# erhant/halo2-vectordb

Hardware: AMD Instinct MI355X
Metric: constraints/sec, proving hot path (witness+layout+commit MSM+NTT), kmeans k=16 circuit (higher is better)
Workload: dtype u32x8 (BN254 Fr/Fq, 254-bit Montgomery)

## Files before the change

halo2_vectordb_amd/csrc/field.hpp:

```cpp
#pragma once
#include <hip/hip_runtime.h>
#include <stdint.h>

#define HD __host__ __device__ __forceinline__

namespace vdb {

struct alignas(16) u256 {
  uint32_t w[8];
};

struct FrParams {
  static constexpr uint32_t P[8] = {0xf0000001u, 0x43e1f593u, 0x79b97091u, 0x2833e848u, 0x8181585du, 0xb85045b6u, 0xe131a029u, 0x30644e72u};
  static constexpr uint32_t R1[8] = {0x4ffffffbu, 0xac96341cu, 0x9f60cd29u, 0x36fc7695u, 0x7879462eu, 0x666ea36fu, 0x9a07df2fu, 0x0e0a77c1u};
  static constexpr uint32_t R2[8] = {0xae216da7u, 0x1bb8e645u, 0xe35c59e3u, 0x53fe3ab1u, 0x53bb8085u, 0x8c49833du, 0x7f4e44a5u, 0x0216d0b1u};
  static constexpr uint32_t INV = 0xefffffffu;
  static constexpr uint32_t P29[9] = {0x10000001u, 0x1f0fac9fu, 0x0e5c2450u, 0x07d090f3u, 0x1585d283u, 0x02db40c0u, 0x00a6e141u, 0x0e5c2634u, 0x0030644eu};
  static constexpr uint32_t INV29 = 0x0fffffffu;
};
struct FqParams {
  static constexpr uint32_t P[8] = {0xd87cfd47u, 0x3c208c16u, 0x6871ca8du, 0x97816a91u, 0x8181585du, 0xb85045b6u, 0xe131a029u, 0x30644e72u};
  static constexpr uint32_t R1[8] = {0xc58f0d9du, 0xd35d438du, 0xf5c70b3du, 0x0a78eb28u, 0x7879462cu, 0x666ea36fu, 0x9a07df2fu, 0x0e0a77c1u};
  static constexpr uint32_t R2[8] = {0x538afa89u, 0xf32cfc5bu, 0xd44501fbu, 0xb5e71911u, 0x0a417ff6u, 0x47ab1effu, 0xcab8351fu, 0x06d89f71u};
  static constexpr uint32_t INV = 0xe4866389u;
// ... 274 lines not shown
  uint64_t acc = 0;
#pragma unroll
  for (int k = 7; k < 18; k++) {
#pragma unroll
    for (int i = (k > 8 ? k - 8 : 0); i <= (k < 8 ? k : 8); i++) mad64(acc, WQ[i], V[k - i]);
    if (k >= 9) q[k - 9] = k < 17 ? ((uint32_t)acc & MASK) : (uint32_t)acc;
    acc >>= 29;
  }
  acc = 0;
#pragma unroll
  for (int k = 0; k < 9; k++) {
#pragma unroll
    for (int i = 0; i <= k; i++) {
      mad64(acc, W[i], V[k - i]);
      mad64(acc, q[i], NP[k - i]);
    }
    out[k] = (uint32_t)acc & MASK;
    acc >>= 29;
  }
#endif
}

template <class M>
HD void mont_sqr_core29(uint32_t out[9], const uint32_t A[9]) {
#if defined(__HIP_DEVICE_COMPILE__)
  uint32_t D[9];
#pragma unroll
  for (int j = 0; j < 9; j++) D[j] = A[j] << 1;
  asm(
#include "core29_sqr.inc"
// ... 216 lines not shown
```

halo2_vectordb_amd/csrc/gen_core29.py:

```python
#!/usr/bin/env python3
ACC = 30


def emit(name, pairs_of, n_arrays):
    O = lambda i: f"%{i}"
    base_p = 9 + 9 * n_arrays
    P = lambda j: f"%{base_p + j}"
    INV = f"%{base_p + 9}"
    acc, lo = f"v[{ACC}:{ACC + 1}]", f"v{ACC}"
    L, first = [], True
    for k in range(18):
        terms = list(pairs_of(k))
        js = range(1, k + 1) if k < 9 else range(k - 8, 9)
        terms += [(O(k - j), P(j)) for j in js]
        for x, y in terms:
            L.append(f"v_mad_u64_u32 {acc}, vcc, {x}, {y}, {0 if first else acc}")
            first = False
        if k < 9:
            L += [f"v_mul_lo_u32 {O(k)}, {lo}, {INV}", f"v_and_b32 {O(k)}, 0x1fffffff, {O(k)}", f"v_mad_u64_u32 {acc}, vcc, {O(k)}, {P(0)}, {acc}"]
        else:
            L.append(f"v_and_b32 {O(k - 9)}, 0x1fffffff, {lo}" if k < 17 else f"v_mov_b32 {O(k - 9)}, {lo}")
        if k < 17:
            L.append(f"v_lshrrev_b64 {acc}, 29, {acc}")
    with open(name, "w") as f:
# ... 32 lines not shown
            L.append(f"v_mad_u64_u32 {acc}, vcc, {W(i)}, {V(k - i)}, {0 if first else acc}")
            first = False
            L.append(f"v_mad_u64_u32 {acc}, vcc, {Q(i)}, {NP(k - i)}, {acc}")
        L.append(f"v_and_b32 {T(k)}, 0x1fffffff, {lo}")
        if k < 8:
            L.append(f"v_lshrrev_b64 {acc}, 29, {acc}")
    with open(name, "w") as f:
        f.write(f"// generated by gen_core29.py — {len(L)} instructions\n")
        f.write("\n".join('"%s\\n\\t"' % x for x in L) + "\n")
    return len(L)


print(emit_shoup("core29_shoup.inc"))


def emit_redc(name):
    O = lambda i: f"%{i}"
    T = lambda i: f"%{9 + i}"
    P = lambda j: f"%{18 + j}"
    INV = "%27"
    acc, lo = f"v[{ACC}:{ACC + 1}]", f"v{ACC}"
    L = []
    for k in range(18):
        if k < 9:
            L.append(f"v_mad_u64_u32 {acc}, vcc, {T(k)}, 1, {0 if k == 0 else acc}")
        js = range(1, k + 1) if k < 9 else range(k - 8, 9)
        for j in js:
            L.append(f"v_mad_u64_u32 {acc}, vcc, {O(k - j)}, {P(j)}, {acc}")
        if k < 9:
            L += [f"v_mul_lo_u32 {O(k)}, {lo}, {INV}", f"v_and_b32 {O(k)}, 0x1fffffff, {O(k)}", f"v_mad_u64_u32 {acc}, vcc, {O(k)}, {P(0)}, {acc}"]
# ... 12 lines not shown
```

halo2_vectordb_amd/csrc/limb9.hpp:

```cpp
#pragma once
#include <math.h>

#include "field.hpp"

namespace vdb {

struct L9 {
  uint32_t l[9];
};
HD L9 l9_split(const u256& a) {
  L9 r;
#pragma unroll
  for (int k = 0; k < 9; k++) {
    int pb = 29 * k, wb = pb >> 5, ob = pb & 31;
    uint32_t lo = a.w[wb];
    uint32_t hi = wb + 1 < 8 ? a.w[wb + 1 < 8 ? wb + 1 : 0] : 0u;
    r.l[k] = ob ? ((lo >> ob) | (hi << (32 - ob))) : lo;
    if (k < 8) r.l[k] &= 0x1fffffffu;
  }
  return r;
}
HD L9 l9_split32(const u256& a) {
  L9 r;
  r.l[0] = (a.w[0] << 5) & 0x1fffffffu;
// ... 79 lines not shown
  const u256 p = mod_p<Fr>();
  u256 r = w;
#pragma unroll
  for (int k = 8; k >= 0; k--) {
    uint32_t d = 0;
    for (int j = 28; j >= 0; j--) {
      u256 s, t;
      u256_add(s, r, r);
      const uint32_t borrow = u256_sub(t, s, p);
      r = borrow ? s : t;
      d |= (borrow ^ 1u) << j;
    }
    out[9 + k] = d;
  }
}
template <class M>
HD L9 l9_mul2(const L9& a1, const L9& b1, const L9& a2, const L9& b2) {
  L9 r;
  mont_core29_2<M>(r.l, a1.l, b1.l, a2.l, b2.l);
  return r;
}
template <class M>
HD L9 l9_sqr(const L9& a) {
  L9 r;
  mont_sqr_core29<M>(r.l, a.l);
  return r;
}
template <class M>
HD u256 l9_canon(const L9& t) {
  return lazy_canon<M>(l9_pack(t));
// ... 32 lines not shown
#pragma unroll
  for (int k = 0; k < 9; k++) {
    const uint32_t nk = (k == 0 ? 0x20000000u : 0x1fffffffu) - FrParams::P29[k];
    acc += (uint64_t)x.l[k] + (uint64_t)q * nk;
    x.l[k] = (uint32_t)acc & 0x1fffffffu;
    acc >>= 29;
  }
  u256 v = l9_pack(x), t, p2, pp = mod_p<Fr>();
  u256_add(p2, pp, pp);
  uint32_t keep = u256_sub(t, v, p2);
#pragma unroll
  for (int i = 0; i < 8; i++) v.w[i] = keep ? v.w[i] : t.w[i];
  return lazy_canon<Fr>(v);
}

}
```

halo2_vectordb_amd/csrc/ntt.hip:

```cpp
#include <type_traits>
#include <vector>

#include "common.hpp"
#include "limb9.hpp"
#include "shoup_tables.hpp"

namespace vdb {

#define NTT_THREADS 256
#define NTT_TILE 1024
#define NTT_MAX_PASSES 4
#define NTT_DEFAULT_COLGROUP 0x7fffffffu

struct NttPass {
  uint32_t log_n, S, log_inner, logG;
  uint32_t nprev;
  uint32_t prevS[NTT_MAX_PASSES];
  uint32_t first;
  uint32_t coset;
  uint32_t vslots;
  const u256* in_tab[4];
  uint32_t coset_out;
  uint32_t scale;
  uint32_t s0;
// ... 65 lines not shown
template <uint32_t CS, uint32_t s, uint32_t step, class F>
__device__ __forceinline__ void ntt_static_steps(F&& f) {
  if constexpr (s < CS) {
    f(std::integral_constant<uint32_t, s>{}, std::integral_constant<uint32_t, step>{});
    ntt_static_steps<CS, (s + 1 < CS ? s + 2 : s + 1), step + 1>(f);
  }
}
constexpr uint32_t ntt_spec_sh_res_log(uint32_t cs, bool sa) { return cs == 8 ? 0u : (sa ? 1u : 2u); }
template <bool LAST, bool VS = false, uint32_t CS = 0, uint32_t CS0 = 0, uint32_t CREN = 0, bool SA = false>
__global__ __launch_bounds__(NTT_THREADS) void k_ntt_pass(const u256* __restrict__ in, u256* __restrict__ out,
                                                         const u256* __restrict__ tw, const u256* __restrict__ tw_inter, NttPass p,
                                                         uint32_t tiles_per_col) {
  extern __shared__ uint4 smem[];
  constexpr bool SPEC = CS > 0;
  static_assert(!SA || ((CS == 8 || CS == 9) && !VS), "SA: the 256- and 512-point instantiations, not the virtual-column one");
  const uint32_t S = SPEC ? CS : p.S, P_logG = SPEC ? 10u - CS : p.logG, P_s0 = SPEC ? CS0 : p.s0, P_ren_mask = SPEC ? CREN : p.ren_mask;
  const uint32_t P_sh_res_log = SPEC ? ntt_spec_sh_res_log(CS, SA) : p.sh_res_log, P_sh_ns = SPEC ? ((1u << (CS ? CS - 1 : 0)) >> ntt_spec_sh_res_log(CS, SA)) : p.sh_ns;
  const int32_t P_sh_max_s = SPEC ? (int32_t)CS - 2 - (int32_t)ntt_spec_sh_res_log(CS, SA) : p.sh_max_s;
  const bool P_shoup = SPEC ? true : p.sh_tab != nullptr, P_blk0 = SPEC ? true : p.blk0 != 0;
  const uint32_t m = 1u << S, G = 1u << P_logG, T = m * G;
  const uint32_t row = m + 1, NE = G * row, NW = SA ? 0u : (m / 2 ? m / 2 : 1);
  L9Planes D, W;
  D.a = smem;
  D.b = D.a + NE;
  W.a = D.b + NE;
  W.b = W.a + NW;
  const uint32_t NS = P_shoup ? P_sh_ns : 0;
  L9Planes WS, WQ;
  WS.a = W.b + NW;
  WS.b = WS.a + NS;
  WQ.a = WS.b + NS;
// ... 75 lines not shown
    if (!LAST) {
      g = e & (G - 1);
      j = e >> P_logG;
    } else {
      j = e & (mload - 1);
      g = e / mload;
    }
    uint64_t idx = base + j * jstride + g * gstride;
    L9 v;
    if (!p.first || idx < p.in_len) {
      v = l9_split(from_src ? colsrc_fetch(csrc, idx, 1ull << p.log_n, p.n_blind) : ld256(cin + idx));
      if constexpr (VS) {
        v = l9_mul(v, l9_split(ld256(ctab + idx)));
      } else if (SA && p.coset) {
        const uint32_t r3 = (uint32_t)(idx % 3);
        if (r3 == 1) v = l9_mul_shoup<Fr>(v, kconst(p.zsh[1]), kconst(p.zsh[1] + 9));
        else if (r3 == 2) v = l9_mul_shoup<Fr>(v, kconst(p.zsh[2]), kconst(p.zsh[2] + 9));
        else if (p.coset == 2) v = l9_mul_shoup<Fr>(v, kconst(p.zsh[0]), kconst(p.zsh[0] + 9));
      } else if (p.coset) {
        uint32_t r3 = (uint32_t)(idx % 3);
        if (r3 == 1) v = l9_mul(v, Z1);
        else if (r3 == 2) v = l9_mul(v, Z2);
        else if (p.coset == 2) v = l9_mul(v, Z0);
      }
    } else {
#pragma unroll
      for (int k = 0; k < 9; k++) v.l[k] = 0;
    }
    for (uint32_t rep = 0; rep < (1u << P_s0); rep++) lds_put(D, g * row + j + rep * mload, v);
  }
  __syncthreads();
  L9 r2w, r2q;
  auto do_step = [&](auto s_c, auto step_c) {
// ... 8 lines not shown
        for (uint32_t t = tid; t < T / 4; t += NTT_THREADS) {
          uint32_t g, r, blk;
          if (S2) {
            const uint32_t lb = P_logG + lh1;
            blk = ((t >> lb) + blockIdx.x + (blockIdx.x >> 8)) & 3u;
            g = (t >> lh1) & (G - 1);
            r = t & (h2 - 1);
          } else {
            const uint32_t gi = t & ((m >> 2) - 1);
            g = t >> (S - 2);
            r = gi & (h2 - 1);
            blk = gi >> lh1;
          }
          const uint32_t j0 = g * row + (blk << (logh + 1)) + r;
          L9 x0 = lds_get(D, j0), x1 = lds_get(D, j0 + h2), x2 = lds_get(D, j0 + h), x3 = lds_get(D, j0 + h + h2);
          if (REN) {
            l9_renorm(x0);
            l9_renorm(x1);
            l9_renorm(x2);
            l9_renorm(x3);
          }
          if (FIRST) {
            L9 a0 = l9_add(x0, x2), a2 = l9_sub(x0, x2, p.ckp);
            L9 a1 = l9_add(x1, x3), a3 = l9_sub(x1, x3, p.ckp);
            l9_carry(a1);
            L9 t3;
            if (SA) {
              const uint32_t iq = (m >> 2) >> P_sh_res_log;
              t3 = l9_mul_shoup<Fr>(a3, lds_get(WS, iq), lds_get(WQ, iq));
            } else {
// ... 65 lines not shown
      } else {
        if (ren) radix4(F_{}, T_{}, F_{}, F_{});
        else if (s2) radix4(F_{}, F_{}, F_{}, T_{});
        else radix4(F_{}, F_{}, F_{}, F_{});
      }
    } else {
      for (uint32_t b = tid; b < T / 2; b += NTT_THREADS) {
        const uint32_t g = b >> (S - 1), pj = b & ((m >> 1) - 1);
        const uint32_t r = pj & (h - 1), blk = pj >> logh, j0 = (blk << (logh + 1)) + r;
        const uint32_t a0 = g * row + j0, a1 = a0 + h;
        L9 u = lds_get(D, a0), v = lds_get(D, a1);
        if (ren) {
          l9_renorm(u);
          l9_renorm(v);
        }
        if (SA) v = l9_mul_shoup<Fr>(v, r2w, r2q);
        else if (s) v = l9_mul(v, lds_get(W, bitrev_s(blk, s) << logh));
        lds_put(D, a0, l9_add(u, v));
        lds_put(D, a1, l9_sub(u, v, p.ckp));
      }
    }
    __syncthreads();
  };
  if constexpr (SPEC) {
    ntt_static_steps<CS, CS0, 0>(do_step);
  } else {
    uint32_t step = 0;
    for (uint32_t s = P_s0; s < S; step++) {
      do_step(s, step);
      s += (s + 1 < S) ? 2 : 1;
    }
  }
  L9 FIN, ZO1, ZO2;
  if (LAST && p.scale) FIN = l9_split(p.fin);
// ... 16 lines not shown
          const uint4 r0 = rp[0], r1 = rp[1], r2 = rp[2], r3 = rp[3], r4 = rp[4];
          trw[it] = L9{{r0.x, r0.y, r0.z, r0.w, r1.x, r1.y, r1.z, r1.w, r2.x}};
          trq[it] = L9{{r2.y, r2.z, r2.w, r3.x, r3.y, r3.z, r3.w, r4.x, r4.y}};
        } else {
          twv[it] = ld256(tw_inter + ex);
        }
      }
    }
  }
#pragma unroll
  for (uint32_t it = 0; it < EPT; it++) {
    const uint32_t e = tid + it * NTT_THREADS;
    if (e >= T) break;
    uint32_t g = e & (G - 1), q = e >> P_logG;
    L9 v = lds_get(D, g * row + bitrev_s(q, S));
    if (p.ren_out) l9_renorm(v);
    if (!LAST) {
      if constexpr (SA) v = l9_mul_shoup<Fr>(v, trw[it], trq[it]);
      else v = l9_mul(v, l9_split(twv[it]));
      st256(cout + base + (uint64_t)q * jstride + g, l9_pack(v));
    } else {
      uint64_t pos;
      if (p.nprev == 0) {
        pos = q;
      } else {
        pos = (uint64_t)q0_base + g;
        uint32_t r = rdig;
        uint32_t shift = 0;
        for (uint32_t l = 0; l < p.nprev; l++) shift += p.prevS[l];
        for (int l = (int)p.nprev - 1; l >= 1; l--) {
          shift -= p.prevS[l];
          uint32_t ql = r & ((1u << p.prevS[l]) - 1);
          r >>= p.prevS[l];
          pos += (uint64_t)ql << shift;
        }
        pos += (uint64_t)q << (p.log_n - S);
      }
      if (p.scale) {
        v = l9_mul(v, FIN);
        const uint32_t r3 = p.coset_out ? (uint32_t)(pos % 3) : 0u;
        if (r3) v = l9_mul(v, r3 == 1 ? ZO1 : ZO2);
        st256(cout + pos, l9_canon(v));
      } else {
        const uint32_t r3 = p.coset_out ? (uint32_t)(pos % 3) : 0u;
        st256(cout + pos, r3 ? l9_canon(l9_mul(v, r3 == 1 ? ZO1 : ZO2)) : l9_canon_wide(v));
      }
    }
  }
}

__global__ __launch_bounds__(256) void k_twiddles(u256* __restrict__ tw, u256 omega, u256 m32, uint64_t n, uint32_t chunk) {
  uint64_t t = (uint64_t)blockIdx.x * blockDim.x + threadIdx.x;
  uint64_t lo = t * chunk;
// ... 21 lines not shown
  uint64_t threads = (n + chunk - 1) / chunk;
  {
    VDB_PROF("k_twiddles");
    hipLaunchKernelGGL(k_twiddles, dim3((unsigned)((threads + 255) / 256)), dim3(256), 0, c.stream, tw, omega, factor, n, chunk);
  }
  e = hipGetLastError();
  if (e != hipSuccess) {
    *err = hip_fail(e, "k_twiddles", __FILE__, __LINE__);
    (void)hipFree(tw);
    return nullptr;
  }
  c.twiddles[key] = tw;
  return tw;
}

static const uint32_t* get_shoup_table(uint32_t log_n, const u256& omega, uint32_t S, uint32_t res_log, int* err) {
  Context& c = ctx();
  Context::TwKey key{log_n | (S << 8) | (res_log << 16) | 0x40000000u, omega};
  auto it = c.twiddles.find(key);
  if (it != c.twiddles.end()) return reinterpret_cast<const uint32_t*>(it->second);
  const std::vector<uint32_t> tab = shoup_stage_entries(log_n, omega, S, res_log);
  uint32_t* d = nullptr;
  hipError_t e = hipMalloc(&d, tab.size() * sizeof(uint32_t));
  if (e != hipSuccess) {
    *err = hip_fail(e, "hipMalloc(shoup table)", __FILE__, __LINE__);
    return nullptr;
  }
  e = hipMemcpy(d, tab.data(), tab.size() * sizeof(uint32_t), hipMemcpyHostToDevice);
  if (e != hipSuccess) {
    *err = hip_fail(e, "hipMemcpy(shoup table)", __FILE__, __LINE__);
    (void)hipFree(d);
    return nullptr;
  }
  c.twiddles[key] = reinterpret_cast<u256*>(d);
  return d;
}

__global__ __launch_bounds__(256) void k_shoup_records(const u256* __restrict__ tw, uint64_t n, u256 inv32, uint4* __restrict__ rec) {
  const uint64_t e = (uint64_t)blockIdx.x * blockDim.x + threadIdx.x;
  if (e >= n) return;
  uint32_t o[20];
  shoup_record_of_tw(ld256(tw + e), inv32, o);
#pragma unroll
  for (int i = 0; i < 5; i++) rec[5 * e + i] = make_uint4(o[4 * i], o[4 * i + 1], o[4 * i + 2], o[4 * i + 3]);
}
static const uint4* get_shoup_records(uint32_t log_n, const u256& omega, bool scaled, const u256* tw, int* err) {
  Context& c = ctx();
  Context::TwKey key{log_n | (scaled ? 0x80000000u : 0u) | 0x20000000u, omega};
  auto it = c.twiddles.find(key);
  if (it != c.twiddles.end()) return reinterpret_cast<const uint4*>(it->second);
  const uint64_t n = 1ull << log_n;
  uint4* d = nullptr;
  hipError_t e = hipMalloc(&d, n * 5 * sizeof(uint4));
  if (e != hipSuccess) {
    *err = hip_fail(e, "hipMalloc(shoup records)", __FILE__, __LINE__);
    return nullptr;
  }
// ... 185 lines not shown
        return spec_on && L > 1 && p.S == cs && p.s0 == cs0 && p.ren_mask == cren && p.logG == 10 - cs && p.blk0;
      };
      static const bool shoup_all = !(getenv("VDB_NTT_SHOUP_ALL") && getenv("VDB_NTT_SHOUP_ALL")[0] == '0');
      const bool sa = shoup_all && shoup_on && !vs && log_n <= 22 &&
                      (spec_shape(8, 0, 4) || spec_shape(9, 0, 20) || (!last && spec_shape(9, 2, 4)));
      size_t lds = (size_t)(G * (m + 1) + (sa ? 0 : (m / 2 ? m / 2 : 1))) * (2 * sizeof(uint4) + sizeof(uint32_t));
      p.sh_tab = nullptr;
      p.sh_res_log = p.sh_ns = 0;
      p.sh_max_s = -1;
      if (shoup_on && S[l] >= 4) {
        const size_t room = (160 * 1024) / 3;
        uint32_t rl = 0;
        while (rl + 2 < S[l] && lds + (size_t)((m / 2) >> rl) * 72 > room) rl++;
        const int32_t max_s = (int32_t)S[l] - 2 - (int32_t)rl;
        if (lds + (size_t)((m / 2) >> rl) * 72 <= room && max_s >= 1) {
          p.sh_tab = get_shoup_table(log_n, omega, S[l], rl, &err);
          if (!p.sh_tab) return err;
          p.sh_res_log = rl;
          p.sh_ns = (m / 2) >> rl;
          p.sh_max_s = max_s;
          lds += (size_t)p.sh_ns * 72;
        }
      }
      dim3 grid((unsigned)(nc * tiles));
      if (lds > 64 * 1024) {
        bool& raised = c.ntt_lds_raised;
        if (!raised) {
          VDB_HIP(hipFuncSetAttribute((const void*)k_ntt_pass<true>, hipFuncAttributeMaxDynamicSharedMemorySize, 96 * 1024));
          VDB_HIP(hipFuncSetAttribute((const void*)k_ntt_pass<false>, hipFuncAttributeMaxDynamicSharedMemorySize, 96 * 1024));
          VDB_HIP(hipFuncSetAttribute((const void*)k_ntt_pass<true, true>, hipFuncAttributeMaxDynamicSharedMemorySize, 96 * 1024));
          VDB_HIP(hipFuncSetAttribute((const void*)k_ntt_pass<false, true>, hipFuncAttributeMaxDynamicSharedMemorySize, 96 * 1024));
          raised = true;
        }
      }
      const u256* twi = last ? tw : (l == 0 ? tw_scaled : tw);
      auto spec = [&](uint32_t cs, uint32_t cs0, uint32_t cren, bool sa_) {
        const uint32_t rl = ntt_spec_sh_res_log(cs, sa_);
        return spec_shape(cs, cs0, cren) && p.sh_tab && p.sh_res_log == rl && p.sh_ns == ((1u << (cs - 1)) >> rl) && p.sh_max_s == (int32_t)cs - 2 - (int32_t)rl;
      };
      if (sa) {
        if (!spec(p.S, p.s0, p.ren_mask, true)) {
          set_error("ntt: SA plan does not match its instantiation");
          return VDB_ERR_ARG;
        }
        if (S[l] & 1) {
          p.sh2_tab = get_shoup_table(log_n, omega, S[l], 0, &err);
          if (!p.sh2_tab) return err;
        }
        if (!last) {
          p.tw_rec = get_shoup_records(log_n, omega, twi != tw, twi, &err);
          if (!p.tw_rec) return err;
        }
        for (int t = 0; t < 3; t++) shoup_const_of_mont(zc[t], p.zsh[t]);
      }
#define NTT_LAUNCH(...) hipLaunchKernelGGL((k_ntt_pass<__VA_ARGS__>), grid, dim3(NTT_THREADS), lds, c.stream, src, out, tw, twi, p, tiles)
      {
        VDB_PROF("k_ntt_pass");
        if (last) {
          if (vs) NTT_LAUNCH(true, true);
          else if (sa && p.S == 8) NTT_LAUNCH(true, false, 8, 0, 4, true);
          else if (sa) NTT_LAUNCH(true, false, 9, 0, 20, true);
          else if (spec(8, 0, 4, false)) NTT_LAUNCH(true, false, 8, 0, 4);
          else if (spec(9, 0, 20, false)) NTT_LAUNCH(true, false, 9, 0, 20);
          else NTT_LAUNCH(true, false);
        } else {
          if (vs && spec(8, 0, 4, false)) NTT_LAUNCH(false, true, 8, 0, 4);
          else if (vs) NTT_LAUNCH(false, true);
          else if (sa && p.S == 8) NTT_LAUNCH(false, false, 8, 0, 4, true);
// ... 214 lines not shown
```

halo2_vectordb_amd/csrc/shoup_tables.hpp:

```cpp
#pragma once
#include <vector>

#include "limb9.hpp"

namespace vdb {

inline void shoup_const_of_mont(const u256& mont, uint32_t out[18]) { shoup_pair29(from_mont<Fr>(mont), out); }

inline std::vector<uint32_t> shoup_stage_entries(uint32_t log_n, const u256& omega, uint32_t S, uint32_t res_log) {
  const uint32_t m = 1u << S, ns = (m / 2) >> res_log;
  std::vector<uint32_t> tab((size_t)ns * 18);
  const u256 step = mont_pow<Fr>(omega, u256_from_u64(((uint64_t)1 << (log_n - S)) << res_log));
  u256 cur = mont_one<Fr>();
  for (uint32_t j = 0; j < ns; j++) {
    shoup_const_of_mont(cur, &tab[18 * (size_t)j]);
    cur = fr_mul(cur, step);
  }
  return tab;
}

HD void shoup_record_of_tw(const u256& t, const u256& inv32, uint32_t out[20]) {
  shoup_pair29(from_mont<Fr>(fr_mul(t, inv32)), out);
  out[18] = out[19] = 0;
}

}
```

Baseline: 1.869 billion.

## Use signed balanced 29-bit limbs in SA NTT butterflies to drop modular corrections

Adds a signed-limb Shoup multiply (v_mad_i64_i32 with a bias), balanced-digit twiddle tables, and signed subtraction without modulus offset in the SA NTT passes. Butterflies now use plain limb subtraction plus cheap arithmetic-shift carry and renorm steps instead of offset-based subtraction and unsigned renormalisation. A wide signed canonicalisation runs at the output. This is meant to cut per-butterfly correction work, at the risk of limb-range overflow and correctness issues in the signed bounds analysis.

After: 1.878 billion (median of 6 runs). Within noise of the previous version (+0.5%).

```diff
diff --git a/halo2_vectordb_amd/csrc/core29_shoup_s.inc b/halo2_vectordb_amd/csrc/core29_shoup_s.inc
--- /dev/null
+++ b/halo2_vectordb_amd/csrc/core29_shoup_s.inc
@@ -0,0 +1,179 @@
+"v_mad_i64_i32 v[30:31], vcc, %36, %25, %54\n\t"
+"v_mad_i64_i32 v[30:31], vcc, %37, %24, v[30:31]\n\t"
+"v_mad_i64_i32 v[30:31], vcc, %38, %23, v[30:31]\n\t"
+"v_mad_i64_i32 v[30:31], vcc, %39, %22, v[30:31]\n\t"
+"v_mad_i64_i32 v[30:31], vcc, %40, %21, v[30:31]\n\t"
+"v_mad_i64_i32 v[30:31], vcc, %41, %20, v[30:31]\n\t"
+"v_mad_i64_i32 v[30:31], vcc, %42, %19, v[30:31]\n\t"
+"v_mad_i64_i32 v[30:31], vcc, %43, %18, v[30:31]\n\t"
+"v_ashrrev_i64 v[30:31], 29, v[30:31]\n\t"
+"v_mad_i64_i32 v[30:31], vcc, %36, %26, v[30:31]\n\t"
+"v_mad_i64_i32 v[30:31], vcc, %37, %25, v[30:31]\n\t"
+"v_mad_i64_i32 v[30:31], vcc, %38, %24, v[30:31]\n\t"
+"v_mad_i64_i32 v[30:31], vcc, %39, %23, v[30:31]\n\t"
+"v_mad_i64_i32 v[30:31], vcc, %40, %22, v[30:31]\n\t"
+"v_mad_i64_i32 v[30:31], vcc, %41, %21, v[30:31]\n\t"
+"v_mad_i64_i32 v[30:31], vcc, %42, %20, v[30:31]\n\t"
+"v_mad_i64_i32 v[30:31], vcc, %43, %19, v[30:31]\n\t"
+"v_mad_i64_i32 v[30:31], vcc, %44, %18, v[30:31]\n\t"
+"v_ashrrev_i64 v[30:31], 29, v[30:31]\n\t"
+"v_mad_i64_i32 v[30:31], vcc, %37, %26, v[30:31]\n\t"
+"v_mad_i64_i32 v[30:31], vcc, %38, %25, v[30:31]\n\t"
+"v_mad_i64_i32 v[30:31], vcc, %39, %24, v[30:31]\n\t"
+"v_mad_i64_i32 v[30:31], vcc, %40, %23, v[30:31]\n\t"
+"v_mad_i64_i32 v[30:31], vcc, %41, %22, v[30:31]\n\t"
+"v_mad_i64_i32 v[30:31], vcc, %42, %21, v[30:31]\n\t"
+"v_mad_i64_i32 v[30:31], vcc, %43, %20, v[30:31]\n\t"
+"v_mad_i64_i32 v[30:31], vcc, %44, %19, v[30:31]\n\t"
+"v_and_b32 %9, 0x1fffffff, v30\n\t"
+"v_ashrrev_i64 v[30:31], 29, v[30:31]\n\t"
+"v_mad_i64_i32 v[30:31], vcc, %38, %26, v[30:31]\n\t"
+"v_mad_i64_i32 v[30:31], vcc, %39, %25, v[30:31]\n\t"
+"v_mad_i64_i32 v[30:31], vcc, %40, %24, v[30:31]\n\t"
+"v_mad_i64_i32 v[30:31], vcc, %41, %23, v[30:31]\n\t"
+"v_mad_i64_i32 v[30:31], vcc, %42, %22, v[30:31]\n\t"
+"v_mad_i64_i32 v[30:31], vcc, %43, %21, v[30:31]\n\t"
+"v_mad_i64_i32 v[30:31], vcc, %44, %20, v[30:31]\n\t"
+"v_and_b32 %10, 0x1fffffff, v30\n\t"
+"v_ashrrev_i64 v[30:31], 29, v[30:31]\n\t"
+"v_mad_i64_i32 v[30:31], vcc, %39, %26, v[30:31]\n\t"
+"v_mad_i64_i32 v[30:31], vcc, %40, %25, v[30:31]\n\t"
+"v_mad_i64_i32 v[30:31], vcc, %41, %24, v[30:31]\n\t"
+"v_mad_i64_i32 v[30:31], vcc, %42, %23, v[30:31]\n\t"
+"v_mad_i64_i32 v[30:31], vcc, %43, %22, v[30:31]\n\t"
+"v_mad_i64_i32 v[30:31], vcc, %44, %21, v[30:31]\n\t"
+"v_and_b32 %11, 0x1fffffff, v30\n\t"
+"v_ashrrev_i64 v[30:31], 29, v[30:31]\n\t"
+"v_mad_i64_i32 v[30:31], vcc, %40, %26, v[30:31]\n\t"
+"v_mad_i64_i32 v[30:31], vcc, %41, %25, v[30:31]\n\t"
+"v_mad_i64_i32 v[30:31], vcc, %42, %24, v[30:31]\n\t"
+"v_mad_i64_i32 v[30:31], vcc, %43, %23, v[30:31]\n\t"
+"v_mad_i64_i32 v[30:31], vcc, %44, %22, v[30:31]\n\t"
+"v_and_b32 %12, 0x1fffffff, v30\n\t"
+"v_ashrrev_i64 v[30:31], 29, v[30:31]\n\t"
+"v_mad_i64_i32 v[30:31], vcc, %41, %26, v[30:31]\n\t"
+"v_mad_i64_i32 v[30:31], vcc, %42, %25, v[30:31]\n\t"
+"v_mad_i64_i32 v[30:31], vcc, %43, %24, v[30:31]\n\t"
+"v_mad_i64_i32 v[30:31], vcc, %44, %23, v[30:31]\n\t"
+"v_and_b32 %13, 0x1fffffff, v30\n\t"
+"v_ashrrev_i64 v[30:31], 29, v[30:31]\n\t"
+"v_mad_i64_i32 v[30:31], vcc, %42, %26, v[30:31]\n\t"
+"v_mad_i64_i32 v[30:31], vcc, %43, %25, v[30:31]\n\t"
+"v_mad_i64_i32 v[30:31], vcc, %44, %24, v[30:31]\n\t"
+"v_and_b32 %14, 0x1fffffff, v30\n\t"
+"v_ashrrev_i64 v[30:31], 29, v[30:31]\n\t"
+"v_mad_i64_i32 v[30:31], vcc, %43, %26, v[30:31]\n\t"
+"v_mad_i64_i32 v[30:31], vcc, %44, %25, v[30:31]\n\t"
+"v_and_b32 %15, 0x1fffffff, v30\n\t"
+"v_ashrrev_i64 v[30:31], 29, v[30:31]\n\t"
+"v_mad_i64_i32 v[30:31], vcc, %44, %26, v[30:31]\n\t"
+"v_and_b32 %16, 0x1fffffff, v30\n\t"
+"v_ashrrev_i64 v[30:31], 29, v[30:31]\n\t"
+"v_mov_b32 %17, v30\n\t"
+"v_mad_i64_i32 v[30:31], vcc, %27, %18, 0\n\t"
+"v_mad_i64_i32 v[30:31], vcc, %9, %45, v[30:31]\n\t"
+"v_and_b32 %0, 0x1fffffff, v30\n\t"
+"v_ashrrev_i64 v[30:31], 29, v[30:31]\n\t"
+"v_mad_i64_i32 v[30:31], vcc, %27, %19, v[30:31]\n\t"
+"v_mad_i64_i32 v[30:31], vcc, %9, %46, v[30:31]\n\t"
+"v_mad_i64_i32 v[30:31], vcc, %28, %18, v[30:31]\n\t"
+"v_mad_i64_i32 v[30:31], vcc, %10, %45, v[30:31]\n\t"
+"v_and_b32 %1, 0x1fffffff, v30\n\t"
+"v_ashrrev_i64 v[30:31], 29, v[30:31]\n\t"
+"v_mad_i64_i32 v[30:31], vcc, %27, %20, v[30:31]\n\t"
+"v_mad_i64_i32 v[30:31], vcc, %9, %47, v[30:31]\n\t"
+"v_mad_i64_i32 v[30:31], vcc, %28, %19, v[30:31]\n\t"
+"v_mad_i64_i32 v[30:31], vcc, %10, %46, v[30:31]\n\t"
+"v_mad_i64_i32 v[30:31], vcc, %29, %18, v[30:31]\n\t"
+"v_mad_i64_i32 v[30:31], vcc, %11, %45, v[30:31]\n\t"
+"v_and_b32 %2, 0x1fffffff, v30\n\t"
+"v_ashrrev_i64 v[30:31], 29, v[30:31]\n\t"
+"v_mad_i64_i32 v[30:31], vcc, %27, %21, v[30:31]\n\t"
+"v_mad_i64_i32 v[30:31], vcc, %9, %48, v[30:31]\n\t"
+"v_mad_i64_i32 v[30:31], vcc, %28, %20, v[30:31]\n\t"
+"v_mad_i64_i32 v[30:31], vcc, %10, %47, v[30:31]\n\t"
+"v_mad_i64_i32 v[30:31], vcc, %29, %19, v[30:31]\n\t"
+"v_mad_i64_i32 v[30:31], vcc, %11, %46, v[30:31]\n\t"
+"v_mad_i64_i32 v[30:31], vcc, %30, %18, v[30:31]\n\t"
+"v_mad_i64_i32 v[30:31], vcc, %12, %45, v[30:31]\n\t"
+"v_and_b32 %3, 0x1fffffff, v30\n\t"
+"v_ashrrev_i64 v[30:31], 29, v[30:31]\n\t"
+"v_mad_i64_i32 v[30:31], vcc, %27, %22, v[30:31]\n\t"
+"v_mad_i64_i32 v[30:31], vcc, %9, %49, v[30:31]\n\t"
+"v_mad_i64_i32 v[30:31], vcc, %28, %21, v[30:31]\n\t"
+"v_mad_i64_i32 v[30:31], vcc, %10, %48, v[30:31]\n\t"
+"v_mad_i64_i32 v[30:31], vcc, %29, %20, v[30:31]\n\t"
+"v_mad_i64_i32 v[30:31], vcc, %11, %47, v[30:31]\n\t"
+"v_mad_i64_i32 v[30:31], vcc, %30, %19, v[30:31]\n\t"
+"v_mad_i64_i32 v[30:31], vcc, %12, %46, v[30:31]\n\t"
+"v_mad_i64_i32 v[30:31], vcc, %31, %18, v[30:31]\n\t"
+"v_mad_i64_i32 v[30:31], vcc, %13, %45, v[30:31]\n\t"
+"v_and_b32 %4, 0x1fffffff, v30\n\t"
+"v_ashrrev_i64 v[30:31], 29, v[30:31]\n\t"
+"v_mad_i64_i32 v[30:31], vcc, %27, %23, v[30:31]\n\t"
+"v_mad_i64_i32 v[30:31], vcc, %9, %50, v[30:31]\n\t"
+"v_mad_i64_i32 v[30:31], vcc, %28, %22, v[30:31]\n\t"
+"v_mad_i64_i32 v[30:31], vcc, %10, %49, v[30:31]\n\t"
+"v_mad_i64_i32 v[30:31], vcc, %29, %21, v[30:31]\n\t"
+"v_mad_i64_i32 v[30:31], vcc, %11, %48, v[30:31]\n\t"
+"v_mad_i64_i32 v[30:31], vcc, %30, %20, v[30:31]\n\t"
+"v_mad_i64_i32 v[30:31], vcc, %12, %47, v[30:31]\n\t"
+"v_mad_i64_i32 v[30:31], vcc, %31, %19, v[30:31]\n\t"
+"v_mad_i64_i32 v[30:31], vcc, %13, %46, v[30:31]\n\t"
+"v_mad_i64_i32 v[30:31], vcc, %32, %18, v[30:31]\n\t"
+"v_mad_i64_i32 v[30:31], vcc, %14, %45, v[30:31]\n\t"
+"v_and_b32 %5, 0x1fffffff, v30\n\t"
+"v_ashrrev_i64 v[30:31], 29, v[30:31]\n\t"
+"v_mad_i64_i32 v[30:31], vcc, %27, %24, v[30:31]\n\t"
+"v_mad_i64_i32 v[30:31], vcc, %9, %51, v[30:31]\n\t"
+"v_mad_i64_i32 v[30:31], vcc, %28, %23, v[30:31]\n\t"
+"v_mad_i64_i32 v[30:31], vcc, %10, %50, v[30:31]\n\t"
+"v_mad_i64_i32 v[30:31], vcc, %29, %22, v[30:31]\n\t"
+"v_mad_i64_i32 v[30:31], vcc, %11, %49, v[30:31]\n\t"
+"v_mad_i64_i32 v[30:31], vcc, %30, %21, v[30:31]\n\t"
+"v_mad_i64_i32 v[30:31], vcc, %12, %48, v[30:31]\n\t"
+"v_mad_i64_i32 v[30:31], vcc, %31, %20, v[30:31]\n\t"
+"v_mad_i64_i32 v[30:31], vcc, %13, %47, v[30:31]\n\t"
+"v_mad_i64_i32 v[30:31], vcc, %32, %19, v[30:31]\n\t"
+"v_mad_i64_i32 v[30:31], vcc, %14, %46, v[30:31]\n\t"
+"v_mad_i64_i32 v[30:31], vcc, %33, %18, v[30:31]\n\t"
+"v_mad_i64_i32 v[30:31], vcc, %15, %45, v[30:31]\n\t"
+"v_and_b32 %6, 0x1fffffff, v30\n\t"
+"v_ashrrev_i64 v[30:31], 29, v[30:31]\n\t"
+"v_mad_i64_i32 v[30:31], vcc, %27, %25, v[30:31]\n\t"
+"v_mad_i64_i32 v[30:31], vcc, %9, %52, v[30:31]\n\t"
+"v_mad_i64_i32 v[30:31], vcc, %28, %24, v[30:31]\n\t"
+"v_mad_i64_i32 v[30:31], vcc, %10, %51, v[30:31]\n\t"
+"v_mad_i64_i32 v[30:31], vcc, %29, %23, v[30:31]\n\t"
+"v_mad_i64_i32 v[30:31], vcc, %11, %50, v[30:31]\n\t"
+"v_mad_i64_i32 v[30:31], vcc, %30, %22, v[30:31]\n\t"
+"v_mad_i64_i32 v[30:31], vcc, %12, %49, v[30:31]\n\t"
+"v_mad_i64_i32 v[30:31], vcc, %31, %21, v[30:31]\n\t"
+"v_mad_i64_i32 v[30:31], vcc, %13, %48, v[30:31]\n\t"
+"v_mad_i64_i32 v[30:31], vcc, %32, %20, v[30:31]\n\t"
+"v_mad_i64_i32 v[30:31], vcc, %14, %47, v[30:31]\n\t"
+"v_mad_i64_i32 v[30:31], vcc, %33, %19, v[30:31]\n\t"
+"v_mad_i64_i32 v[30:31], vcc, %15, %46, v[30:31]\n\t"
+"v_mad_i64_i32 v[30:31], vcc, %34, %18, v[30:31]\n\t"
+"v_mad_i64_i32 v[30:31], vcc, %16, %45, v[30:31]\n\t"
+"v_and_b32 %7, 0x1fffffff, v30\n\t"
+"v_ashrrev_i64 v[30:31], 29, v[30:31]\n\t"
+"v_mad_i64_i32 v[30:31], vcc, %27, %26, v[30:31]\n\t"
+"v_mad_i64_i32 v[30:31], vcc, %9, %53, v[30:31]\n\t"
+"v_mad_i64_i32 v[30:31], vcc, %28, %25, v[30:31]\n\t"
+"v_mad_i64_i32 v[30:31], vcc, %10, %52, v[30:31]\n\t"
+"v_mad_i64_i32 v[30:31], vcc, %29, %24, v[30:31]\n\t"
+"v_mad_i64_i32 v[30:31], vcc, %11, %51, v[30:31]\n\t"
+"v_mad_i64_i32 v[30:31], vcc, %30, %23, v[30:31]\n\t"
+"v_mad_i64_i32 v[30:31], vcc, %12, %50, v[30:31]\n\t"
+"v_mad_i64_i32 v[30:31], vcc, %31, %22, v[30:31]\n\t"
+"v_mad_i64_i32 v[30:31], vcc, %13, %49, v[30:31]\n\t"
+"v_mad_i64_i32 v[30:31], vcc, %32, %21, v[30:31]\n\t"
+"v_mad_i64_i32 v[30:31], vcc, %14, %48, v[30:31]\n\t"
+"v_mad_i64_i32 v[30:31], vcc, %33, %20, v[30:31]\n\t"
+"v_mad_i64_i32 v[30:31], vcc, %15, %47, v[30:31]\n\t"
+"v_mad_i64_i32 v[30:31], vcc, %34, %19, v[30:31]\n\t"
+"v_mad_i64_i32 v[30:31], vcc, %16, %46, v[30:31]\n\t"
+"v_mad_i64_i32 v[30:31], vcc, %35, %18, v[30:31]\n\t"
+"v_mad_i64_i32 v[30:31], vcc, %17, %45, v[30:31]\n\t"
+"v_and_b32 %8, 0x1fffffff, v30\n\t"
diff --git a/halo2_vectordb_amd/csrc/field.hpp b/halo2_vectordb_amd/csrc/field.hpp
--- a/halo2_vectordb_amd/csrc/field.hpp
+++ b/halo2_vectordb_amd/csrc/field.hpp
@@ -312,6 +312,46 @@
     for (int i = 0; i <= k; i++) {
       mad64(acc, W[i], V[k - i]);
       mad64(acc, q[i], NP[k - i]);
+    }
+    out[k] = (uint32_t)acc & MASK;
+    acc >>= 29;
+  }
+#endif
+}
+
+template <class M>
+HD void shoup_core29_s(uint32_t out[9], const uint32_t V[9], const uint32_t W[9], const uint32_t WQ[9]) {
+  constexpr int64_t BIAS = -(int64_t)13 * ((int64_t)1 << 52);
+#if defined(__HIP_DEVICE_COMPILE__)
+  uint32_t q[9];
+  asm(
+#include "core29_shoup_s.inc"
+      : VDB_CORE29_OUT(out), VDB_CORE29_OUT(q)
+      : VDB_CORE29_IN(V), VDB_CORE29_IN(W), VDB_CORE29_IN(WQ), "s"((0x20000000u) - M::P29[0]), "s"(0x1fffffffu - M::P29[1]), "s"(0x1fffffffu - M::P29[2]),
+        "s"(0x1fffffffu - M::P29[3]), "s"(0x1fffffffu - M::P29[4]), "s"(0x1fffffffu - M::P29[5]), "s"(0x1fffffffu - M::P29[6]), "s"(0x1fffffffu - M::P29[7]),
+        "s"(0x1fffffffu - M::P29[8]), "s"(BIAS)
+      : VDB_CORE29_CLOBBER);
+#else
+  constexpr uint32_t MASK = 0x1fffffffu;
+  auto smad = [](int64_t& acc, uint32_t a, uint32_t b) { acc += (int64_t)(int32_t)a * (int64_t)(int32_t)b; };
+  uint32_t q[9], NP[9];
+#pragma unroll
+  for (int k = 0; k < 9; k++) NP[k] = (k == 0 ? 0x20000000u : 0x1fffffffu) - M::P29[k];
+  int64_t acc = BIAS;
+#pragma unroll
+  for (int k = 7; k < 18; k++) {
+#pragma unroll
+    for (int i = (k > 8 ? k - 8 : 0); i <= (k < 8 ? k : 8); i++) smad(acc, WQ[i], V[k - i]);
+    if (k >= 9) q[k - 9] = k < 17 ? ((uint32_t)acc & MASK) : (uint32_t)acc;
+    acc >>= 29;
+  }
+  acc = 0;
+#pragma unroll
+  for (int k = 0; k < 9; k++) {
+#pragma unroll
+    for (int i = 0; i <= k; i++) {
+      smad(acc, W[i], V[k - i]);
+      smad(acc, q[i], NP[k - i]);
     }
     out[k] = (uint32_t)acc & MASK;
     acc >>= 29;
diff --git a/halo2_vectordb_amd/csrc/gen_core29.py b/halo2_vectordb_amd/csrc/gen_core29.py
--- a/halo2_vectordb_amd/csrc/gen_core29.py
+++ b/halo2_vectordb_amd/csrc/gen_core29.py
@@ -1,4 +1,6 @@
 #!/usr/bin/env python3
+import sys
+
 ACC = 30
 
 
@@ -70,6 +72,43 @@
 print(emit_shoup("core29_shoup.inc"))
 
 
+def emit_shoup_s(name):
+    T = lambda i: f"%{i}"
+    Q = lambda i: f"%{9 + i}"
+    V = lambda i: f"%{18 + i}"
+    W = lambda i: f"%{27 + i}"
+    WQ = lambda i: f"%{36 + i}"
+    NP = lambda i: f"%{45 + i}"
+    BIAS = "%54"
+    acc, lo = f"v[{ACC}:{ACC + 1}]", f"v{ACC}"
+    L, first = [], True
+    for k in range(7, 18):
+        for i in range(max(0, k - 8), min(8, k) + 1):
+            L.append(f"v_mad_i64_i32 {acc}, vcc, {WQ(i)}, {V(k - i)}, {BIAS if first else acc}")
+            first = False
+        if k >= 9:
+            L.append(f"v_and_b32 {Q(k - 9)}, 0x1fffffff, {lo}" if k < 17 else f"v_mov_b32 {Q(k - 9)}, {lo}")
+        if k < 17:
+            L.append(f"v_ashrrev_i64 {acc}, 29, {acc}")
+    first = True
+    for k in range(9):
+        for i in range(k + 1):
+            L.append(f"v_mad_i64_i32 {acc}, vcc, {W(i)}, {V(k - i)}, {0 if first else acc}")
+            first = False
+            L.append(f"v_mad_i64_i32 {acc}, vcc, {Q(i)}, {NP(k - i)}, {acc}")
+        L.append(f"v_and_b32 {T(k)}, 0x1fffffff, {lo}")
+        if k < 8:
+            L.append(f"v_ashrrev_i64 {acc}, 29, {acc}")
+    with open(name, "w") as f:
+        f.write(f"// generated by gen_core29.py — {len(L)} instructions\n")
+        f.write("\n".join('"%s\\n\\t"' % x for x in L) + "\n")
+    return len(L)
+
+
+if "--signed" in sys.argv:
+    print(emit_shoup_s("core29_shoup_s.inc"))
+
+
 def emit_redc(name):
     O = lambda i: f"%{i}"
     T = lambda i: f"%{9 + i}"
diff --git a/halo2_vectordb_amd/csrc/limb9.hpp b/halo2_vectordb_amd/csrc/limb9.hpp
--- a/halo2_vectordb_amd/csrc/limb9.hpp
+++ b/halo2_vectordb_amd/csrc/limb9.hpp
@@ -117,6 +117,50 @@
     out[9 + k] = d;
   }
 }
+HD L9 l9s_sub(const L9& a, const L9& t) {
+  L9 r;
+#pragma unroll
+  for (int k = 0; k < 9; k++) r.l[k] = a.l[k] - t.l[k];
+  return r;
+}
+HD void l9s_renorm(L9& x) {
+  int32_t c[8];
+#pragma unroll
+  for (int k = 0; k < 8; k++) c[k] = (int32_t)x.l[k] >> 29;
+#pragma unroll
+  for (int k = 0; k < 8; k++) x.l[k] &= 0x1fffffffu;
+#pragma unroll
+  for (int k = 1; k < 9; k++) x.l[k] += (uint32_t)c[k - 1];
+}
+HD void l9s_carry(L9& x) {
+#pragma unroll
+  for (int k = 0; k < 8; k++) {
+    x.l[k + 1] += (uint32_t)((int32_t)x.l[k] >> 29);
+    x.l[k] &= 0x1fffffffu;
+  }
+}
+HD void l9_balance(uint32_t l[9]) {
+  uint32_t carry = 0;
+#pragma unroll
+  for (int k = 0; k < 8; k++) {
+    uint32_t d = l[k] + carry;
+    carry = d >= (1u << 28) ? 1u : 0u;
+    l[k] = d - (carry << 29);
+  }
+  l[8] += carry;
+}
+HD void shoup_pair29_s(const u256& w, uint32_t out[18]) {
+  shoup_pair29(w, out);
+  l9_balance(out);
+  l9_balance(out + 9);
+}
+template <class M>
+HD L9 l9s_mul_shoup(const L9& v, const L9& w, const L9& wq) {
+  L9 r;
+  shoup_core29_s<M>(r.l, v.l, w.l, wq.l);
+  return r;
+}
+
 template <class M>
 HD L9 l9_mul2(const L9& a1, const L9& b1, const L9& a2, const L9& b2) {
   L9 r;
@@ -179,4 +223,25 @@
   return lazy_canon<Fr>(v);
 }
 
-}
+HD u256 l9s_canon_wide(L9 x) {
+  constexpr uint32_t MU = 2840127191u;
+  constexpr uint32_t D = 0x30644eu + 1u;
+  const uint32_t e = x.l[8] + (uint32_t)((int32_t)x.l[7] >> 29) + (32u * D - 1u);
+  const int32_t qs = (int32_t)((uint32_t)(((uint64_t)(e << 3) * MU) >> 32) >> 24) - 33;
+  int64_t acc = 0;
+#pragma unroll
+  for (int k = 0; k < 9; k++) {
+    const uint32_t nk = (k == 0 ? 0x20000000u : 0x1fffffffu) - FrParams::P29[k];
+    acc += (int64_t)(int32_t)x.l[k] + (int64_t)qs * (int64_t)nk;
+    x.l[k] = (uint32_t)acc & 0x1fffffffu;
+    acc >>= 29;
+  }
+  u256 v = l9_pack(x), t, p2, pp = mod_p<Fr>();
+  u256_add(p2, pp, pp);
+  uint32_t keep = u256_sub(t, v, p2);
+#pragma unroll
+  for (int i = 0; i < 8; i++) v.w[i] = keep ? v.w[i] : t.w[i];
+  return lazy_canon<Fr>(v);
+}
+
+}
diff --git a/halo2_vectordb_amd/csrc/ntt.hip b/halo2_vectordb_amd/csrc/ntt.hip
--- a/halo2_vectordb_amd/csrc/ntt.hip
+++ b/halo2_vectordb_amd/csrc/ntt.hip
@@ -103,7 +103,7 @@
   extern __shared__ uint4 smem[];
   constexpr bool SPEC = CS > 0;
   static_assert(!SA || ((CS == 8 || CS == 9) && !VS), "SA: the 256- and 512-point instantiations, not the virtual-column one");
-  const uint32_t S = SPEC ? CS : p.S, P_logG = SPEC ? 10u - CS : p.logG, P_s0 = SPEC ? CS0 : p.s0, P_ren_mask = SPEC ? CREN : p.ren_mask;
+  const uint32_t S = SPEC ? CS : p.S, P_logG = SPEC ? 10u - CS : p.logG, P_s0 = SPEC ? CS0 : p.s0, P_ren_mask = SA ? 0u : (SPEC ? CREN : p.ren_mask);
   const uint32_t P_sh_res_log = SPEC ? ntt_spec_sh_res_log(CS, SA) : p.sh_res_log, P_sh_ns = SPEC ? ((1u << (CS ? CS - 1 : 0)) >> ntt_spec_sh_res_log(CS, SA)) : p.sh_ns;
   const int32_t P_sh_max_s = SPEC ? (int32_t)CS - 2 - (int32_t)ntt_spec_sh_res_log(CS, SA) : p.sh_max_s;
   const bool P_shoup = SPEC ? true : p.sh_tab != nullptr, P_blk0 = SPEC ? true : p.blk0 != 0;
@@ -209,9 +209,9 @@
         v = l9_mul(v, l9_split(ld256(ctab + idx)));
       } else if (SA && p.coset) {
         const uint32_t r3 = (uint32_t)(idx % 3);
-        if (r3 == 1) v = l9_mul_shoup<Fr>(v, kconst(p.zsh[1]), kconst(p.zsh[1] + 9));
-        else if (r3 == 2) v = l9_mul_shoup<Fr>(v, kconst(p.zsh[2]), kconst(p.zsh[2] + 9));
-        else if (p.coset == 2) v = l9_mul_shoup<Fr>(v, kconst(p.zsh[0]), kconst(p.zsh[0] + 9));
+        if (r3 == 1) v = l9s_mul_shoup<Fr>(v, kconst(p.zsh[1]), kconst(p.zsh[1] + 9));
+        else if (r3 == 2) v = l9s_mul_shoup<Fr>(v, kconst(p.zsh[2]), kconst(p.zsh[2] + 9));
+        else if (p.coset == 2) v = l9s_mul_shoup<Fr>(v, kconst(p.zsh[0]), kconst(p.zsh[0] + 9));
       } else if (p.coset) {
         uint32_t r3 = (uint32_t)(idx % 3);
         if (r3 == 1) v = l9_mul(v, Z1);
@@ -250,6 +250,53 @@
           }
           const uint32_t j0 = g * row + (blk << (logh + 1)) + r;
           L9 x0 = lds_get(D, j0), x1 = lds_get(D, j0 + h2), x2 = lds_get(D, j0 + h), x3 = lds_get(D, j0 + h + h2);
+          if constexpr (SA) {
+            if (FIRST) {
+              const L9 a0 = l9_add(x0, x2), a2 = l9s_sub(x0, x2), a1 = l9_add(x1, x3), a3 = l9s_sub(x1, x3);
+              const uint32_t iq = (m >> 2) >> P_sh_res_log;
+              const L9 t3 = l9s_mul_shoup<Fr>(a3, lds_get(WS, iq), lds_get(WQ, iq));
+              x0 = l9_add(a0, a1);
+              x1 = l9s_sub(a0, a1);
+              x2 = l9_add(a2, t3);
+              x3 = l9s_sub(a2, t3);
+            } else if (S2 && blk == 0) {
+              if (step > 0) {
+                l9s_carry(x0);
+                l9s_carry(x1);
+                l9s_carry(x2);
+                l9s_carry(x3);
+              }
+              const L9 a0 = l9_add(x0, x2), a2 = l9s_sub(x0, x2), a1 = l9_add(x1, x3), a3 = l9s_sub(x1, x3);
+              const uint32_t iq = (m >> 2) >> P_sh_res_log;
+              const L9 t3 = l9s_mul_shoup<Fr>(a3, lds_get(WS, iq), lds_get(WQ, iq));
+              x0 = l9_add(a0, a1);
+              x1 = l9s_sub(a0, a1);
+              x2 = l9_add(a2, t3);
+              x3 = l9s_sub(a2, t3);
+            } else {
+              if (step > 0) {
+                l9s_renorm(x0);
+                l9s_renorm(x1);
+              }
+              const uint32_t e = bitrev_s(blk, s) << logh, rl = P_sh_res_log;
+              const uint32_t i0 = e >> rl, i1 = (e >> 1) >> rl, i2 = ((e >> 1) + (m >> 2)) >> rl;
+              const L9 ws = lds_get(WS, i0), wq = lds_get(WQ, i0);
+              const L9 t2 = l9s_mul_shoup<Fr>(x2, ws, wq), t3 = l9s_mul_shoup<Fr>(x3, ws, wq);
+              const L9 a0 = l9_add(x0, t2), a2 = l9s_sub(x0, t2);
+              const L9 a1 = l9_add(x1, t3), a3 = l9s_sub(x1, t3);
+              const L9 u1 = l9s_mul_shoup<Fr>(a1, lds_get(WS, i1), lds_get(WQ, i1));
+              const L9 u3 = l9s_mul_shoup<Fr>(a3, lds_get(WS, i2), lds_get(WQ, i2));
+              x0 = l9_add(a0, u1);
+              x1 = l9s_sub(a0, u1);
+              x2 = l9_add(a2, u3);
+              x3 = l9s_sub(a2, u3);
+            }
+            lds_put(D, j0, x0);
+            lds_put(D, j0 + h2, x1);
+            lds_put(D, j0 + h, x2);
+            lds_put(D, j0 + h + h2, x3);
+            continue;
+          }
           if (REN) {
             l9_renorm(x0);
             l9_renorm(x1);
@@ -345,10 +392,10 @@
           l9_renorm(u);
           l9_renorm(v);
         }
-        if (SA) v = l9_mul_shoup<Fr>(v, r2w, r2q);
+        if (SA) v = l9s_mul_shoup<Fr>(v, r2w, r2q);
         else if (s) v = l9_mul(v, lds_get(W, bitrev_s(blk, s) << logh));
         lds_put(D, a0, l9_add(u, v));
-        lds_put(D, a1, l9_sub(u, v, p.ckp));
+        lds_put(D, a1, SA ? l9s_sub(u, v) : l9_sub(u, v, p.ckp));
       }
     }
     __syncthreads();
@@ -395,9 +442,9 @@
     if (e >= T) break;
     uint32_t g = e & (G - 1), q = e >> P_logG;
     L9 v = lds_get(D, g * row + bitrev_s(q, S));
-    if (p.ren_out) l9_renorm(v);
+    if (!SA && p.ren_out) l9_renorm(v);
     if (!LAST) {
-      if constexpr (SA) v = l9_mul_shoup<Fr>(v, trw[it], trq[it]);
+      if constexpr (SA) v = l9s_mul_shoup<Fr>(v, trw[it], trq[it]);
       else v = l9_mul(v, l9_split(twv[it]));
       st256(cout + base + (uint64_t)q * jstride + g, l9_pack(v));
     } else {
@@ -417,7 +464,11 @@
         }
         pos += (uint64_t)q << (p.log_n - S);
       }
-      if (p.scale) {
+      if constexpr (SA) {
+        const uint32_t r3 = p.coset_out ? (uint32_t)(pos % 3) : 0u;
+        if (r3) v = l9s_mul_shoup<Fr>(v, kconst(p.zsh[3 - r3]), kconst(p.zsh[3 - r3] + 9));
+        st256(cout + pos, r3 ? l9_canon(v) : l9s_canon_wide(v));
+      } else if (p.scale) {
         v = l9_mul(v, FIN);
         const uint32_t r3 = p.coset_out ? (uint32_t)(pos % 3) : 0u;
         if (r3) v = l9_mul(v, r3 == 1 ? ZO1 : ZO2);
@@ -469,12 +520,12 @@
   return tw;
 }
 
-static const uint32_t* get_shoup_table(uint32_t log_n, const u256& omega, uint32_t S, uint32_t res_log, int* err) {
+static const uint32_t* get_shoup_table(uint32_t log_n, const u256& omega, uint32_t S, uint32_t res_log, bool balanced, int* err) {
   Context& c = ctx();
-  Context::TwKey key{log_n | (S << 8) | (res_log << 16) | 0x40000000u, omega};
+  Context::TwKey key{log_n | (S << 8) | (res_log << 16) | 0x40000000u | (balanced ? 0x10000000u : 0u), omega};
   auto it = c.twiddles.find(key);
   if (it != c.twiddles.end()) return reinterpret_cast<const uint32_t*>(it->second);
-  const std::vector<uint32_t> tab = shoup_stage_entries(log_n, omega, S, res_log);
+  const std::vector<uint32_t> tab = shoup_stage_entries(log_n, omega, S, res_log, balanced);
   uint32_t* d = nullptr;
   hipError_t e = hipMalloc(&d, tab.size() * sizeof(uint32_t));
   if (e != hipSuccess) {
@@ -495,7 +546,7 @@
   const uint64_t e = (uint64_t)blockIdx.x * blockDim.x + threadIdx.x;
   if (e >= n) return;
   uint32_t o[20];
-  shoup_record_of_tw(ld256(tw + e), inv32, o);
+  shoup_record_of_tw_s(ld256(tw + e), inv32, o);
 #pragma unroll
   for (int i = 0; i < 5; i++) rec[5 * e + i] = make_uint4(o[4 * i], o[4 * i + 1], o[4 * i + 2], o[4 * i + 3]);
 }
@@ -711,7 +762,7 @@
         while (rl + 2 < S[l] && lds + (size_t)((m / 2) >> rl) * 72 > room) rl++;
         const int32_t max_s = (int32_t)S[l] - 2 - (int32_t)rl;
         if (lds + (size_t)((m / 2) >> rl) * 72 <= room && max_s >= 1) {
-          p.sh_tab = get_shoup_table(log_n, omega, S[l], rl, &err);
+          p.sh_tab = get_shoup_table(log_n, omega, S[l], rl, sa, &err);
           if (!p.sh_tab) return err;
           p.sh_res_log = rl;
           p.sh_ns = (m / 2) >> rl;
@@ -741,14 +792,14 @@
           return VDB_ERR_ARG;
         }
         if (S[l] & 1) {
-          p.sh2_tab = get_shoup_table(log_n, omega, S[l], 0, &err);
+          p.sh2_tab = get_shoup_table(log_n, omega, S[l], 0, true, &err);
           if (!p.sh2_tab) return err;
         }
         if (!last) {
           p.tw_rec = get_shoup_records(log_n, omega, twi != tw, twi, &err);
           if (!p.tw_rec) return err;
         }
-        for (int t = 0; t < 3; t++) shoup_const_of_mont(zc[t], p.zsh[t]);
+        for (int t = 0; t < 3; t++) shoup_const_of_mont_s(zc[t], p.zsh[t]);
       }
 #define NTT_LAUNCH(...) hipLaunchKernelGGL((k_ntt_pass<__VA_ARGS__>), grid, dim3(NTT_THREADS), lds, c.stream, src, out, tw, twi, p, tiles)
       {
diff --git a/halo2_vectordb_amd/csrc/shoup_tables.hpp b/halo2_vectordb_amd/csrc/shoup_tables.hpp
--- a/halo2_vectordb_amd/csrc/shoup_tables.hpp
+++ b/halo2_vectordb_amd/csrc/shoup_tables.hpp
@@ -6,14 +6,16 @@
 namespace vdb {
 
 inline void shoup_const_of_mont(const u256& mont, uint32_t out[18]) { shoup_pair29(from_mont<Fr>(mont), out); }
+inline void shoup_const_of_mont_s(const u256& mont, uint32_t out[18]) { shoup_pair29_s(from_mont<Fr>(mont), out); }
 
-inline std::vector<uint32_t> shoup_stage_entries(uint32_t log_n, const u256& omega, uint32_t S, uint32_t res_log) {
+inline std::vector<uint32_t> shoup_stage_entries(uint32_t log_n, const u256& omega, uint32_t S, uint32_t res_log, bool balanced = false) {
   const uint32_t m = 1u << S, ns = (m / 2) >> res_log;
   std::vector<uint32_t> tab((size_t)ns * 18);
   const u256 step = mont_pow<Fr>(omega, u256_from_u64(((uint64_t)1 << (log_n - S)) << res_log));
   u256 cur = mont_one<Fr>();
   for (uint32_t j = 0; j < ns; j++) {
-    shoup_const_of_mont(cur, &tab[18 * (size_t)j]);
+    if (balanced) shoup_const_of_mont_s(cur, &tab[18 * (size_t)j]);
+    else shoup_const_of_mont(cur, &tab[18 * (size_t)j]);
     cur = fr_mul(cur, step);
   }
   return tab;
@@ -23,5 +25,9 @@
   shoup_pair29(from_mont<Fr>(fr_mul(t, inv32)), out);
   out[18] = out[19] = 0;
 }
+HD void shoup_record_of_tw_s(const u256& t, const u256& inv32, uint32_t out[20]) {
+  shoup_pair29_s(from_mont<Fr>(fr_mul(t, inv32)), out);
+  out[18] = out[19] = 0;
+}
 
 }
```
